# Horizon1026/Feature_Tracker

Hardware: AMD Instinct MI355X
Metric: tracked features/sec (2000 pts, 640x480, 4-lvl pyr) (higher is better)
Workload: dtype f32; 1 GPU; config2: basic KLT inverse, 2000 features/GPU, 640x480, 4-level pyramid, 21x21 patch; parallelism=single GPU

## Files before the change

feature_tracker_amd/csrc/ftk_device.h:

```cpp
#pragma once

#include <hip/hip_runtime.h>
#include <stdint.h>

#include "../../include/ftk.h"

namespace ftk {

constexpr int kWave = 64;

constexpr int kAffineTermsGroupFloats = 4 * 24 + 4;
constexpr int kAffineTermsRoundGroups = 4;

struct DevImage {
    const uint8_t *data;
    int32_t rows;
    int32_t cols;
};

struct KltParams {
    DevImage ref[FTK_MAX_LEVELS];
    DevImage cur[FTK_MAX_LEVELS];
    int32_t n_levels;
    int32_t single_level;
// ... 23 lines not shown
    int32_t half_rows, half_cols;
    float converge;
    float prior[4];
    int32_t consider_luminance;
    int32_t patch_rows, patch_cols, P, Ppad;
    int32_t ex_rows, ex_cols, E;
    int32_t a0_floats;
    uint32_t magic_pc;
    uint32_t magic_pc20;
    uint32_t magic_exc;
    int32_t rwin_rows, rwin_cols;
    int32_t cwin_rows, cwin_cols, cwin_margin;
    uint32_t magic_rwc, magic_cwc;
    uint32_t magic_rwq, magic_cwq;
    int32_t waves_per_feature;
    int32_t px_floats;
    int32_t quad_chain;
    int32_t terms_floats;
    int32_t lssd_chunked;
    int32_t features_per_group;
    int32_t group_lds_stride;
    int32_t pb_enabled;
    int32_t pb_rwin_rows, pb_rwin_cols;
    uint32_t pb_magic_rwc, pb_magic_rwq;
    int32_t pb_cap_r, pb_cap_c;
    int32_t fk_enabled;
    int32_t spill;
    float *spill_base;
    uint32_t spill_stride_floats;
    int32_t tree;
    int32_t scale_recip;
};

__host__ __device__ constexpr uint32_t klt_div_magic(int32_t d) { return d <= 1 ? 0u : (uint32_t)(((1ull << 32) + (uint64_t)d - 1) / (uint64_t)d); }

__host__ __device__ constexpr void klt_fill_geometry(KltParams &p) {
    p.patch_rows = 2 * p.half_rows + 1;
    p.patch_cols = 2 * p.half_cols + 1;
    p.P = p.patch_rows * p.patch_cols;
    p.Ppad = (p.P + 15) & ~15;
    p.ex_rows = p.patch_rows + 2;
    p.ex_cols = p.patch_cols + 2;
    p.E = p.ex_rows * p.ex_cols;
    const int32_t epad = (p.E + 3) & ~3, tables = 12 * (p.patch_rows + p.patch_cols);
    p.a0_floats = epad > tables ? epad : tables;
    p.magic_pc = klt_div_magic(p.patch_cols);
    p.magic_pc20 = (p.patch_cols > 1 && (long long)p.P * p.patch_cols < (1ll << 20) && p.P < (1 << 12))
                       ? (uint32_t)(((1u << 20) + (uint32_t)p.patch_cols - 1) / (uint32_t)p.patch_cols) : 0u;
    p.magic_exc = klt_div_magic(p.ex_cols);
    p.rwin_rows = p.patch_rows + 3;
    p.rwin_cols = (p.patch_cols + 3 + 3) & ~3;
    p.cwin_margin = 2;
    p.cwin_rows = p.rwin_rows + 2 * p.cwin_margin;
    p.cwin_cols = (p.patch_cols + 3 + 2 * p.cwin_margin + 3) & ~3;
    p.magic_rwc = klt_div_magic(p.rwin_cols);
    p.magic_cwc = klt_div_magic(p.cwin_cols);
    p.magic_rwq = klt_div_magic(p.rwin_cols / 4);
    p.magic_cwq = klt_div_magic(p.cwin_cols / 4);
    p.pb_rwin_rows = p.patch_rows + 4;
    p.pb_rwin_cols = (p.patch_cols + 4 + 3) & ~3;
    p.pb_magic_rwc = klt_div_magic(p.pb_rwin_cols);
    p.pb_magic_rwq = klt_div_magic(p.pb_rwin_cols / 4);
    int bits_r = 0, bits_c = 0;
    while ((1 << bits_r) < p.patch_rows + 2) {
        ++bits_r;
    }
    while ((1 << bits_c) < p.patch_cols + 2) {
        ++bits_c;
    }
    p.pb_cap_r = p.patch_rows + 2 + 2 * (bits_r + 3);
    p.pb_cap_c = p.patch_cols + 2 + 2 * (bits_c + 3);
}

hipError_t klt_position_order_launch(const float *ref_uv, int32_t n, const uint32_t *last_table, uint32_t last_call, uint8_t *pred, uint32_t *hist_and_cursor,
                                     int32_t *order, hipStream_t stream);
hipError_t ldlt6_launch(const float *d_a, const float *d_b, float *d_x, int n, hipStream_t stream);

constexpr int kMatchBlock = 256;
constexpr int kMatchRefs = 2;
constexpr int kMatchRowsPerBlock = kMatchBlock * kMatchRefs;
constexpr int kMfmaRows = 64;
constexpr int kMfmaTile = 32;
constexpr int kMfmaMaxTilesPerSplit = 1024;
constexpr long long kSmallMatchWork = 32ll << 20;
constexpr int kSmallMatchRowWork = 24576;
constexpr int kSmallNoIndex = 0xFFFFF;

struct MatchParams {
    const uint32_t *ref_words;
    const uint32_t *cur_words;
    const float *pred_uv;
    const float *cur_uv;
    int32_t *index_pairs;
    unsigned long long *keys;
// ... 371 lines not shown
```

feature_tracker_amd/csrc/klt_basic_kernels.hip:

```cpp
#define FTK_CHAIN_ROUND 4
#include "klt_common.h"
#include "klt_plan.h"

namespace ftk {
namespace {

constexpr int kChunk = 64;
constexpr bool pb_row_chunks(int patch_rows, int patch_cols) {
    if (patch_rows < 1 || patch_cols < 1 || patch_cols > kChunk) {
        return false;
    }
    const int rows_per_chunk = kChunk / patch_cols;
    return (patch_rows + rows_per_chunk - 1) / rows_per_chunk == (patch_rows * patch_cols + kChunk - 1) / kChunk;
}
template <int HR, int HC>
struct PbChunks {
    static constexpr int kRows = HR > 0 && HC > 0 ? 2 * HR + 1 : 0, kCols = HR > 0 && HC > 0 ? 2 * HC + 1 : 0;
    static constexpr bool kByRows = pb_row_chunks(kRows, kCols);
    static constexpr int kRowsPerChunk = kByRows ? kChunk / kCols : 1;
    static constexpr int kCount = kByRows ? (kRows + kRowsPerChunk - 1) / kRowsPerChunk : 0;
    static constexpr bool kLastRowsShort = kCount * kRowsPerChunk > kRows;
};
static_assert(PbChunks<10, 10>::kByRows && PbChunks<10, 10>::kCount == 7 && !PbChunks<10, 10>::kLastRowsShort, "21 x 21: seven chunks of three rows");
static_assert(!PbChunks<6, 6>::kByRows && !PbChunks<5, 5>::kByRows && !PbChunks<0, 0>::kByRows, "13 x 13, 11 x 11 and the run-time geometry stay linear");
constexpr int kRingRow = kChunk + 16;
constexpr int kTerms = 5;
constexpr int kCurQuads = 4;
constexpr int kRefQuads = 3;

__host__ __device__ inline int pb_pad4(int x) { return (x + 3) & ~3; }
__host__ __device__ inline int pb_producers(int waves) { return waves > 1 ? waves - 1 : 1; }
__host__ __device__ inline int pb_ring_slots(int waves) { return waves > 1 ? 2 : 1; }

struct PbLds {
    float4 *rnodes, *cnodes;
    uint4 *ridx, *cidx;
    float4 *ctab;
    float *ring;
    float *lattice;
    float *sol;
    uint32_t *slots;
    uint16_t *ref_win;
    int ref_win_stride;
    uint16_t *cur_win;
};

__host__ __device__ inline int pb_tables(const KltParams &p, int waves) { return p.tree ? waves : pb_producers(waves); }

__host__ __device__ inline size_t pb_lds_bytes(const KltParams &p, int waves) {
    const int np = pb_producers(waves);
    size_t bytes = 16 * (size_t)(p.pb_cap_r + p.pb_cap_c);
    bytes += 16 * (size_t)(p.patch_rows + p.patch_cols);
    bytes += 16 * (size_t)pb_tables(p, waves) * 2 * (p.patch_rows + p.patch_cols);
    bytes += 4 * (size_t)pb_ring_slots(waves) * np * kTerms * kRingRow;
    bytes += 4 * (size_t)pb_pad4(p.pb_cap_r * p.pb_cap_c);
    bytes += 4 * 4 + 4 * 16;
    bytes += 2 * (size_t)2 * pb_pad4(p.pb_rwin_rows * p.pb_rwin_cols);
    bytes += 2 * (size_t)pb_pad4(p.cwin_rows * p.cwin_cols);
    return (bytes + 15) & ~(size_t)15;
}

__device__ __forceinline__ PbLds pb_carve(float4 *base, const KltParams &p, int waves) {
    const int np = pb_producers(waves);
    PbLds c;
    c.rnodes = base;
    c.cnodes = c.rnodes + p.pb_cap_r;
    c.ridx = reinterpret_cast<uint4 *>(c.cnodes + p.pb_cap_c);
    c.cidx = c.ridx + p.patch_rows;
    c.ctab = reinterpret_cast<float4 *>(c.cidx + p.patch_cols);
    c.ring = reinterpret_cast<float *>(c.ctab + pb_tables(p, waves) * 2 * (p.patch_rows + p.patch_cols));
    c.lattice = c.ring + pb_ring_slots(waves) * np * kTerms * kRingRow;
    c.sol = c.lattice + pb_pad4(p.pb_cap_r * p.pb_cap_c);
    c.slots = reinterpret_cast<uint32_t *>(c.sol + 4);
    c.ref_win = reinterpret_cast<uint16_t *>(c.slots + 16);
    c.ref_win_stride = pb_pad4(p.pb_rwin_rows * p.pb_rwin_cols);
    c.cur_win = c.ref_win + 2 * c.ref_win_stride;
    return c;
}

__device__ __forceinline__ float4 node_entry(float x, int limit, int lo, int extent, int pitch) {
    const Axis a = make_axis(x, limit);
    const int rel = (int)((unsigned)a.i0 - (unsigned)lo);
    const bool hit = (unsigned)rel < (unsigned)extent;
    return make_float4(__int_as_float(hit ? rel * pitch : 0), a.sub, a.inv, __int_as_float((a.valid && hit) ? 1 : 0));
}

struct AxisSpec {
    int len, h, limit, lo, extent, pitch, cap;
    float centre;
    float4 *nodes;
    uint4 *idx;
    uint32_t *n_out;
};

__device__ __forceinline__ void build_nodes_pass(int lane, const AxisSpec &A, const AxisSpec &B) {
    const bool is_b = lane >= A.len;
    const int len = is_b ? B.len : A.len;
    const int h = is_b ? B.h : A.h;
// ... 36 lines not shown
        if (t == 0 || t == len - 1) {
            nodes[t == 0 ? 0 : len + 1] = node_entry(t == 0 ? xm : xp, limit, lo, extent, pitch);
        }
        const int im = (t == 0) ? 0 : (needm ? em : t);
        const int ip = (t == len - 1) ? len + 1 : (needp ? ep : t + 2);
        idx[t] = make_uint4((unsigned)(t + 1), (unsigned)im, (unsigned)ip, (v0 && vm && vp) ? 1u : 0u);
        if (t == 0) {
            *(is_b ? B.n_out : A.n_out) = (uint32_t)total;
        }
    }
    if (len == 1 && act) {
        nodes[2] = node_entry(xp, limit, lo, extent, pitch);
    }
    if ((bm | bp) != 0ull) {
        if (needm) {
            nodes[em] = node_entry(xm, limit, lo, extent, pitch);
        }
        if (needp) {
            nodes[ep] = node_entry(xp, limit, lo, extent, pitch);
        }
    }
}

__device__ __forceinline__ float node_tap(const uint16_t *win, int wcols, const float4 &nr, const float4 &nc) {
    const int idx = __float_as_int(nr.x) + __float_as_int(nc.x);
    const unsigned a = win[idx];
    const unsigned bb = win[idx + wcols];
    const float w_tl = nr.z * nc.z;
    const float w_tr = nr.z * nc.y;
    const float w_bl = nr.y * nc.z;
    const float w_br = nr.y * nc.y;
    return w_tl * (float)(a & 0xFFu) + w_tr * (float)(a >> 8) + w_bl * (float)(bb & 0xFFu) + w_br * (float)(bb >> 8);
}

__device__ __forceinline__ void cur_tables(int lane, const KltParams &p, const PbLds &c, float4 *tab, const DevImage &cur, const Win &cw, float cur_u,
                                           float cur_v, int n_c) {
    const int total = p.patch_rows + p.patch_cols;
    for (int t = lane; t < total; t += kWave) {
        const bool is_row = t < p.patch_rows;
        const int d = is_row ? t : t - p.patch_rows;
        const float x = (float)(d - (is_row ? p.half_rows : p.half_cols)) + (is_row ? cur_v : cur_u);
        float4 e = node_entry(x, (is_row ? cur.rows : cur.cols) - 1, is_row ? cw.r_lo : cw.c_lo, is_row ? cw.rows - 1 : cw.cols,
                              is_row ? cw.cols : 1);
        const uint4 id = is_row ? c.ridx[d] : c.cidx[d];
        e.w = __int_as_float(__float_as_int(e.w) & (int)id.w);
        const int mul = is_row ? n_c : 1;
        tab[t] = e;
        tab[total + t] = make_float4(__int_as_float((int)id.x * mul), __int_as_float((int)id.y * mul), __int_as_float((int)id.z * mul), 0.0f);
    }
}

struct PbLane {
    int row, col;
    bool in;
};
struct PbCols {
    float4 c0, c1;
};
template <class G>
__device__ __forceinline__ PbLane pb_lane(int lane) {
    PbLane l = {0, 0, false};
    if constexpr (G::kByRows) {
        constexpr uint32_t kMagic = (1048576 + G::kCols - 1) / G::kCols;
        const int row = (int)(__umul24((uint32_t)lane, kMagic) >> 20);
        l.in = lane < G::kRowsPerChunk * G::kCols;
        l.row = l.in ? row : 0;
        l.col = l.in ? lane - row * G::kCols : 0;
    }
    return l;
}
template <class G>
__device__ __forceinline__ void pb_read_cols(const PbLane &l, const KltParams &p, const float4 *tab, PbCols &cols) {
    if constexpr (G::kByRows) {
        cols.c0 = tab[p.patch_rows + l.col];
        cols.c1 = tab[2 * p.patch_rows + p.patch_cols + l.col];
    }
}

template <class G>
__device__ __forceinline__ bool chunk_products(int lane, int chunk, const KltParams &p, const PbLds &c, const float4 *tab, const Win &cw, const PbLane &l,
                                               const PbCols &cols, float (&prod)[kTerms]) {
    const int tab_total = p.patch_rows + p.patch_cols;
    bool in;
    float4 r0, r1, c0, c1;
    if constexpr (G::kByRows) {
        int prow = wadd(l.row, imul(chunk, G::kRowsPerChunk));
        in = l.in;
        if constexpr (G::kLastRowsShort) {
            in = in && prow < p.patch_rows;
            prow = in ? prow : 0;
        }
        r0 = tab[prow];
        r1 = tab[tab_total + prow];
        c0 = cols.c0;
        c1 = cols.c1;
    } else {
        const int pxi = chunk * kChunk + lane;
        in = pxi < p.P;
        const int pp = in ? pxi : 0;
        int prow, pcol;
        pixel_rc(p, pp, prow, pcol);
        r0 = tab[prow];
        r1 = tab[tab_total + prow];
        c0 = tab[p.patch_rows + pcol];
        c1 = tab[tab_total + p.patch_rows + pcol];
    }
    const float i_cur = node_tap(cw.data, cw.cols, r0, c0);
    const float *lat = c.lattice;
    const int rc = __float_as_int(r1.x), rm = __float_as_int(r1.y), rp = __float_as_int(r1.z);
    const int cc = __float_as_int(c1.x), cm = __float_as_int(c1.y), cp = __float_as_int(c1.z);
    const float left = lat[rc + cm];
    const float right = lat[rc + cp];
    const float top = lat[rm + cc];
    const float bottom = lat[rp + cc];
    const float i_ref = lat[rc + cc];
    const bool ok = in && ((__float_as_int(r0.w) & __float_as_int(c0.w)) != 0);
    const float fx = ok ? right - left : 0.0f;
    const float fy = ok ? bottom - top : 0.0f;
    const float ft = ok ? i_cur - i_ref : 0.0f;
    prod[0] = fx * fx;
    prod[1] = fy * fy;
    prod[2] = fx * fy;
    prod[3] = -(fx * ft);
    prod[4] = -(fy * ft);
    return ok;
}

template <class G>
__device__ __forceinline__ bool produce_chunk(int lane, int chunk, const KltParams &p, const PbLds &c, const float4 *tab, const Win &cw, const PbLane &l,
                                              const PbCols &cols, float *slot) {
    float prod[kTerms];
    const bool ok = chunk_products<G>(lane, chunk, p, c, tab, cw, l, cols, prod);
#pragma unroll
    for (int k = 0; k < kTerms; ++k) {
        slot[k * kRingRow + lane] = prod[k];
    }
    return ok;
}

__device__ __forceinline__ void wave_sum5(float (&v)[kTerms]) {
#pragma unroll
    for (int off = 32; off >= 1; off >>= 1) {
#pragma unroll
        for (int k = 0; k < kTerms; ++k) {
            v[k] += __shfl_xor(v[k], off, kWave);
        }
    }
}

__device__ __forceinline__ uint32_t magic20(int d) {
    uint32_t m = (uint32_t)(1048576.0f / (float)d);
    while (m * (uint32_t)d < 1048576u) {
        ++m;
    }
    return m;
}

constexpr int kWavesPerEu = 4;

__device__ __forceinline__ bool pb_window_inside(const DevImage &im, int r_lo, int c_lo, int wrows, int wcols) {
    return r_lo >= 0 && c_lo >= 0 && r_lo <= im.rows - wrows && c_lo <= im.cols - wcols - 4;
}

__device__ __forceinline__ void pb_sync(bool solo) {
    if (solo) {
        __builtin_amdgcn_fence(__ATOMIC_ACQ_REL, "wavefront");
        __builtin_amdgcn_wave_barrier();
    } else {
        __syncthreads();
    }
}

template <bool SOLO, int HR, int HC, bool TREE>
__global__ void __attribute__((amdgpu_waves_per_eu(kWavesPerEu))) __launch_bounds__(256) klt_basic_inverse_pipelined_kernel(const KltParams p_arg) {
    klt_touch_kernarg<sizeof(KltParams)>();
    KltParams p = p_arg;
    if constexpr (HR > 0 && HC > 0) {
        p.half_rows = HR;
        p.half_cols = HC;
        klt_fill_geometry(p);
    }
    extern __shared__ float4 lds_raw[];
    Blk b;
    uint32_t id;
    float4 *lds_mine = lds_raw;
    uint32_t block = blockIdx.x;
    if (p.sort_iters) {
        if (block == 0) {
            klt_order_block(p.sort_iters, p.sort_order_out, p.n, reinterpret_cast<int *>(lds_raw), p.sort_ref_uv, p_arg.ref[0].cols, p_arg.ref[0].rows, SOLO ? max(p.features_per_group, 1) : 1,
                            p.sched_flags, p.sched_call);
            return;
        }
        block -= 1;
    }
    if (SOLO) {
        b.tid = b.lane = threadIdx.x & (kWave - 1);
        b.nt = kWave;
        b.wave = 0;
        b.nwaves = 1;
        const uint32_t slot = threadIdx.x >> 6;
        id = block * (uint32_t)p.features_per_group + slot;
        lds_mine = lds_raw + (size_t)slot * (p.group_lds_stride >> 4);
    } else {
        b.tid = threadIdx.x;
// ... 60 lines not shown
    const bool last_chunk_short = !G::kByRows && p.P - (n_chunks - 1) * kChunk <= 48;
    const float *const quad_rows = c.ring + min(b.lane >> 2, kTerms - 1) * kRingRow + 4 * (b.lane & 3);

    const float full_ref_u = full_ref.x, full_ref_v = full_ref.y;
    const float scale = p.single_level ? 1.0f : (float)(1 << (p.n_levels - 1));
    float ref_u = full_ref_u, ref_v = full_ref_v, cur_u = in_u, cur_v = in_v;
    if (!p.single_level) {
        const uint32_t k = (uint32_t)(p.n_levels - 1);
        const float inv_scale = __uint_as_float((127u - k) << 23), least = __uint_as_float((1u + k) << 23);
        const bool normal = fabsf(full_ref_u) >= least && fabsf(full_ref_v) >= least && fabsf(in_u) >= least && fabsf(in_v) >= least;
        if (p.scale_recip && wave_ballot(!normal) == 0ull) {
            ref_u = full_ref_u * inv_scale;
            ref_v = full_ref_v * inv_scale;
            cur_u = in_u * inv_scale;
            cur_v = in_v * inv_scale;
        } else {
            ref_u = full_ref_u / scale;
            ref_v = full_ref_v / scale;
            cur_u = in_u / scale;
            cur_v = in_v / scale;
        }
    }

    const int rrows = p.pb_rwin_rows, rcols = p.pb_rwin_cols;
    const int ref_quads_total = rrows * (rcols >> 2), cur_quads_total = p.cwin_rows * (p.cwin_cols >> 2);
    const bool ref_fits = ref_quads_total <= kRefQuads * b.nt, cur_fits = cur_quads_total <= kCurQuads * b.nt;

    int buf = 0;
    int ref_r_lo, ref_c_lo;
    {
        const DevImage ref = p_arg.ref[p.n_levels - 1];
        footprint_origin(p, ref_u, ref_v, ref_r_lo, ref_c_lo);
        stage_any(opaque_blk(b), ref, c.ref_win, ref_r_lo, ref_c_lo, rrows, rcols, p.pb_magic_rwc, p.pb_magic_rwq);
    }
    uint32_t iters = 0;
    float out_u = in_u, out_v = in_v;
    const int base_n_c = p.patch_cols + 2;
    const uint32_t base_magic = (HC > 0) ? (uint32_t)((1048576 + base_n_c - 1) / base_n_c) : magic20(base_n_c);
    for (int level = p.n_levels - 1; level > -1; --level) {
        const DevImage ref = p_arg.ref[level];
        const DevImage cur = p_arg.cur[level];
        set_level_priority(level, younger);
        Win rw, cw;
        rw.data = c.ref_win + buf * c.ref_win_stride;
        rw.rows = rrows;
        rw.cols = rcols;
        rw.r_lo = ref_r_lo;
        rw.c_lo = ref_c_lo;
        int need_r, need_c;
        footprint_origin(p, cur_u, cur_v, need_r, need_c);
        cw.data = c.cur_win;
        cw.r_lo = wadd(need_r, -p.cwin_margin);
        cw.c_lo = wadd(need_c, -p.cwin_margin);
        cw.rows = p.cwin_rows;
        cw.cols = p.cwin_cols;
        win_set_cover(p, cw);
        int nr_lo = 0, nc_lo = 0;
        if (level > 0) {
            footprint_origin(p, ref_u * 2.0f, ref_v * 2.0f, nr_lo, nc_lo);
        }
        const bool cur_async = cur_fits && pb_window_inside(cur, cw.r_lo, cw.c_lo, cw.rows, cw.cols);
        const bool next_async = level > 0 && ref_fits && pb_window_inside(p_arg.ref[level > 0 ? level - 1 : 0], nr_lo, nc_lo, rrows, rcols);
        RawQuads<kCurQuads> qc;
        RawQuads<kRefQuads> qn;
        if (cur_async) {
            issue_quads(qc, b, cur, cw.r_lo, cw.c_lo, cw.rows, cw.cols, p.magic_cwq);
        }
        if (next_async) {
            issue_quads(qn, b, p_arg.ref[level - 1], nr_lo, nc_lo, rrows, rcols, p.pb_magic_rwq);
        }
        if (b.wave == 0) {
            AxisSpec ar = {p.patch_rows, p.half_rows, ref.rows - 1, rw.r_lo, rw.rows - 1, rw.cols, p.pb_cap_r, ref_v, c.rnodes, c.ridx, &c.slots[0]};
            AxisSpec ac = {p.patch_cols, p.half_cols, ref.cols - 1, rw.c_lo, rw.cols, 1, p.pb_cap_c, ref_u, c.cnodes, c.cidx, &c.slots[1]};
            const int lane = opaque(b.lane);
            if (p.patch_rows + p.patch_cols <= kWave) {
                build_nodes_pass(lane, ar, ac);
            } else {
                AxisSpec none = ar;
                none.len = 0;
                build_nodes_pass(lane, ar, none);
                build_nodes_pass(lane, ac, none);
            }
        }
        pb_sync(solo);
        const int n_r = __builtin_amdgcn_readfirstlane((int)c.slots[0]), n_c = __builtin_amdgcn_readfirstlane((int)c.slots[1]);
        {
            const int total = n_r * n_c;
            const uint32_t m = (n_c == base_n_c) ? base_magic : magic20(n_c);
            for (int idx = opaque(b.tid); idx < total; idx += b.nt) {
                const int r = (int)(__umul24((uint32_t)idx, m) >> 20);
                const int cc = idx - imul(r, n_c);
                c.lattice[idx] = node_tap(rw.data, rw.cols, c.rnodes[r], c.cnodes[cc]);
            }
        }
        if (cur_async) {
            store_quads(qc, b, c.cur_win, cw.rows, cw.cols, p.magic_cwq);
        } else {
            stage_any(opaque_blk(b), cur, c.cur_win, cw.r_lo, cw.c_lo, cw.rows, cw.cols, p.magic_cwc, p.magic_cwq);
        }
        if (level > 0) {
            if (next_async) {
                store_quads(qn, b, c.ref_win + (buf ^ 1) * c.ref_win_stride, rrows, rcols, p.pb_magic_rwq);
            } else {
                stage_any(opaque_blk(b), p_arg.ref[level - 1], c.ref_win + (buf ^ 1) * c.ref_win_stride, nr_lo, nc_lo, rrows, rcols, p.pb_magic_rwc, p.pb_magic_rwq);
            }
        }
        pb_sync(solo);

        for (uint32_t iter = 0; iter < p.max_iteration; ++iter) {
            ++iters;
            if (iter > 0 && !win_covers(cw, cur_u, cur_v)) {
                footprint_origin(p, cur_u, cur_v, need_r, need_c);
                const long long nr = need_r, nc = need_c;
                const bool covered = nr >= (long long)cw.r_lo && nr + (2 * p.half_rows + 4) <= (long long)cw.r_lo + cw.rows &&
                                     nc >= (long long)cw.c_lo && nc + (2 * p.half_cols + 4) <= (long long)cw.c_lo + cw.cols + 1;
                if (!covered) {
                    cw.r_lo = wadd(need_r, -p.cwin_margin);
                    cw.c_lo = wadd(need_c, -p.cwin_margin);
                    win_set_cover(p, cw);
                    stage_any(opaque_blk(b), cur, c.cur_win, cw.r_lo, cw.c_lo, cw.rows, cw.cols, p.magic_cwc, p.magic_cwq);
                    pb_sync(solo);
                }
            }
            uint32_t wave_valid = 0;
            float acc = 0.0f;
            PbCols my_cols = {};
            if constexpr (TREE) {
                float part[kTerms] = {0.0f, 0.0f, 0.0f, 0.0f, 0.0f};
                cur_tables(b.lane, p, c, my_tab, cur, cw, cur_u, cur_v, n_c);
                __builtin_amdgcn_wave_barrier();
                pb_read_cols<G>(my_px, p, my_tab, my_cols);
                for (int chunk = b.wave; chunk < n_chunks; chunk += b.nwaves) {
                    float prod[kTerms];
                    const bool ok = chunk_products<G>(b.lane, chunk, p, c, my_tab, cw, my_px, my_cols, prod);
#pragma unroll
                    for (int k = 0; k < kTerms; ++k) {
                        part[k] += prod[k];
                    }
                    wave_valid += (uint32_t)__popcll(wave_ballot(ok));
                }
                wave_sum5(part);
                float *const wave_sums = c.ring;
                if (b.lane == 0) {
// ... 121 lines not shown
        if (p.iters) {
            p.iters[id] = iters;
        }
        tail_report(p, iters, id);
        sched_grid_record(p, full_ref_u, full_ref_v, out_u, out_v, iters);
        if (p.sched_iters) {
            p.sched_iters[id] = iters;
        }
    }
}


}

namespace {
template <int HR, int HC>
KltKernel pick_kernel(bool solo, bool tree) {
    void (*entry)(const KltParams);
    if (tree) {
        entry = solo ? klt_basic_inverse_pipelined_kernel<true, HR, HC, true> : klt_basic_inverse_pipelined_kernel<false, HR, HC, true>;
    } else {
        entry = solo ? klt_basic_inverse_pipelined_kernel<true, HR, HC, false> : klt_basic_inverse_pipelined_kernel<false, HR, HC, false>;
    }
    return {entry, "pipelined", HR, solo, tree, false, false, PbChunks<HR, HC>::kByRows};
}
}

size_t klt_pipelined_feature_lds_bytes(const KltParams &p) { return pb_lds_bytes(p, p.waves_per_feature); }

KltKernel klt_pipelined_pick(const KltParams &p) {
    const bool solo = p.waves_per_feature == 1;
    if (p.half_rows == p.half_cols) {
        KltParams check = p;
        klt_fill_geometry(check);
        const bool same = check.pb_cap_r == p.pb_cap_r && check.pb_cap_c == p.pb_cap_c && check.cwin_rows == p.cwin_rows && check.cwin_cols == p.cwin_cols;
        if (same) {
            switch (p.half_rows) {
                case 5: return pick_kernel<5, 5>(solo, p.tree != 0);
                case 6: return pick_kernel<6, 6>(solo, p.tree != 0);
                case 10: return pick_kernel<10, 10>(solo, p.tree != 0);
                default: break;
            }
        }
    }
    return pick_kernel<0, 0>(solo, p.tree != 0);
}

__global__ void klt_basic_warm_kernel() {}
hipError_t klt_basic_warm(hipStream_t stream) {
    hipLaunchKernelGGL(klt_basic_warm_kernel, dim3(1), dim3(64), 0, stream);
    return hipGetLastError();
}

}
```

feature_tracker_amd/csrc/klt_common.h:

```cpp
#pragma once

#include "ftk_device.h"
#include "klt_sched.h"

#include <limits.h>
#include <math.h>
#include <stddef.h>

#include <type_traits>

namespace ftk {
namespace {



__device__ __forceinline__ int f2i(float x) { return (x >= -2147483648.0f && x < 2147483648.0f) ? (int)x : INT_MIN; }
__device__ __forceinline__ int wadd(int a, int b) { return (int)((unsigned)a + (unsigned)b); }
__device__ __forceinline__ int imul(int a, int b) { return __mul24(a, b); }
__device__ __forceinline__ unsigned long long wave_ballot(bool pred) { return __builtin_amdgcn_ballot_w64(pred); }
__device__ __forceinline__ float floor_from_trunc(float x, int t) {
    const float f = (float)t;
    return (f > x) ? f - 1.0f : f;
}
__device__ __forceinline__ float px(const DevImage &im, int row, int col) { return (float)im.data[__umul24((unsigned)row, (unsigned)im.cols) + (unsigned)col]; }
// ... 929 lines not shown
template <bool kBlocks64 = false>
__device__ __forceinline__ float chain_quads_row(float acc, const float *quad_row, int n16) {
    return chain_quads_strided<kBlocks64>(acc, reinterpret_cast<const float4 *>(quad_row), n16, 4);
}

constexpr int kChunkPixels = 64;
constexpr int kChunkRow = kChunkPixels + 4;

__device__ __forceinline__ void pixel_rc(const KltParams &p, int pxi, int &prow, int &pcol) {
    if (p.magic_pc20 != 0) {
        prow = (int)(__umul24((unsigned)pxi, p.magic_pc20) >> 20);
    } else {
        prow = (p.patch_cols == 1) ? pxi : (int)__umulhi((unsigned)pxi, p.magic_pc);
    }
    pcol = pxi - imul(prow, p.patch_cols);
}


__device__ __forceinline__ void footprint_origin(const KltParams &p, float u, float v, int &r_lo, int &c_lo) {
    r_lo = __builtin_amdgcn_readfirstlane(wadd(f2i(floorf(v)), -(p.half_rows + 1)));
    c_lo = __builtin_amdgcn_readfirstlane(wadd(f2i(floorf(u)), -(p.half_cols + 1)));
}

__device__ __forceinline__ void win_set_cover(const KltParams &p, Win &w) {
    const bool small = (unsigned)(w.r_lo + (1 << 22)) < (1u << 23) && (unsigned)(w.c_lo + (1 << 22)) < (1u << 23);
    w.cover[0] = small ? (float)(w.r_lo + p.half_rows + 1) : 1.0f;
    w.cover[1] = small ? (float)(w.r_lo + w.rows - p.half_rows - 3) : 0.0f;
    w.cover[2] = small ? (float)(w.c_lo + p.half_cols + 1) : 1.0f;
    w.cover[3] = small ? (float)(w.c_lo + w.cols - p.half_cols - 2) : 0.0f;
}

__device__ __forceinline__ bool win_covers(const Win &w, float u, float v) {
    const float fu = floorf(u), fv = floorf(v);
    return fv >= w.cover[0] && fv <= w.cover[1] && fu >= w.cover[2] && fu <= w.cover[3];
}

__device__ __forceinline__ uint16_t window_element(const DevImage &im, int r_lo, int c_lo, int idx, int wcols, uint32_t magic_cols) {
    const int r = (int)__umulhi((unsigned)idx, magic_cols);
    const int c = idx - imul(r, wcols);
    const int ir = clampi(wadd(r_lo, r), 0, im.rows - 1);
    const int ic = wadd(c_lo, c);
    const int ic0 = clampi(ic, 0, im.cols - 1);
    const int ic1 = clampi(wadd(ic, 1), 0, im.cols - 1);
    const unsigned row_off = __umul24((unsigned)ir, (unsigned)im.cols);
    return (uint16_t)((unsigned)im.data[row_off + (unsigned)ic0] | ((unsigned)im.data[row_off + (unsigned)ic1] << 8));
}

constexpr int kStageBatch = 4;

__device__ __forceinline__ void stage_elements(const Blk &b, const DevImage &im, uint16_t *dst, int r_lo, int c_lo, int wcols, uint32_t magic_cols,
                                               int total) {
    for (int base = 0; base < total; base += b.nt * kStageBatch) {
        uint16_t v[kStageBatch];
#pragma unroll
        for (int k = 0; k < kStageBatch; ++k) {
// ... 101 lines not shown
}

template <int N>
__device__ __forceinline__ void store_quads(const RawQuads<N> &q, const Blk &b, uint16_t *dst, int wrows, int wcols, uint32_t magic_quads) {
    const int quads = wcols >> 2;
    const int total = wrows * quads;
    const int tid = opaque(b.tid);
#pragma unroll
    for (int k = 0; k < N; ++k) {
        const int idx = tid + k * b.nt;
        if (idx < total) {
            const int r = (quads == 1) ? idx : (int)__umulhi((unsigned)idx, magic_quads);
            const int qq = idx - imul(r, quads);
            const uint32_t x = q.x[k], y = q.y[k];
            const uint32_t p0 = x & 0xFFFFu;
            const uint32_t p1 = (x >> 8) & 0xFFFFu;
            const uint32_t p2 = x >> 16;
            const uint32_t p3 = __builtin_amdgcn_alignbyte(y, x, 3) & 0xFFFFu;
            *reinterpret_cast<uint2 *>(dst + imul(r, wcols) + 4 * qq) = make_uint2(p0 | (p1 << 16), p2 | (p3 << 16));
        }
    }
}

}


__device__ __forceinline__ uint32_t sched_table_slot(float u, float v) {
    const uint32_t qx = (uint32_t)(int)fminf(fmaxf(u * 0.25f, 0.0f), 1048575.0f), qy = (uint32_t)(int)fminf(fmaxf(v * 0.25f, 0.0f), 1048575.0f);
    return ((qx * 73856093u) ^ (qy * 19349663u)) & (uint32_t)(kSchedTableSize - 1);
}

__device__ __forceinline__ uint32_t sched_prediction(const KltParams &p, float u, float v) {
    const uint32_t word = p.sched_grid[(((p.sched_call - 1u) & 1u) << kSchedTableBits) + sched_table_slot(u, v)];
    return sched_grid_call(word) == sched_grid_tag(p.sched_call - 1u) ? sched_grid_iters(word) : 0u;
}

__device__ __forceinline__ void sched_grid_record(const KltParams &p, float ref_u, float ref_v, float out_u, float out_v, uint32_t iters) {
    if (p.sched_grid != nullptr) {
        const uint32_t word = sched_grid_pack(p.sched_call, iters);
        uint32_t *table = p.sched_grid + sched_table_at(p.sched_call);
        const uint32_t at_ref = sched_table_slot(ref_u, ref_v), at_out = sched_table_slot(out_u, out_v);
        atomicMax(&table[at_ref], word);
        if (at_out != at_ref) {
            atomicMax(&table[at_out], word);
        }
    }
// ... 258 lines not shown
```

feature_tracker_amd/csrc/klt_plan.cpp:

```cpp
#include "klt_plan.h"

#include <algorithm>

namespace ftk {
namespace {
#include "klt_wave_policy.inc"

int policy_bucket(const int *centres, int count, int x) {
    int best = 0;
    for (int i = 1; i < count; ++i) {
        if ((long long)x * x > (long long)centres[i - 1] * centres[i]) {
            best = i;
        }
    }
    return best;
}

int clamp_1_4(int x) { return x < 1 ? 1 : (x > 4 ? 4 : x); }

bool fast_like(int method) { return method != FTK_METHOD_INVERSE && method != FTK_METHOD_DIRECT; }

bool affine_terms(const KltPlanInput &in) { return in.model == FTK_MODEL_AFFINE && !fast_like(in.method); }

int32_t affine_terms_floats(const KltParams &p) {
    return ((p.Ppad / 4 + kAffineTermsRoundGroups - 1) / kAffineTermsRoundGroups) * kAffineTermsRoundGroups * kAffineTermsGroupFloats;
}

int plan_waves(const KltPlanInput &in, int pixels) {
    int waves = klt_policy_waves(in.model, klt_method_class(in.method), in.consider_luminance, in.long_tail, pixels, in.n);
    if (in.tree && waves == 1 && fast_like(in.method) && in.model != FTK_MODEL_LSSD) {
        waves = std::min(4, std::max(2, (pixels + 63) / 64));
    }
    return in.waves != kKltNotSet ? in.waves : clamp_1_4(waves);
}

int plan_group(const KltPlanInput &in, int waves, int measured_best) {
    if (waves != 1) {
        return 1;
    }
    return in.group != kKltNotSet ? in.group : measured_best;
}

KltForm pick_form(const KltPlanInput &in, const KltParams &geometry, int waves) {
    const bool exact_coordinates = in.max_extent < (1 << 23);
    if (in.model == FTK_MODEL_BASIC && in.method == FTK_METHOD_INVERSE && geometry.patch_rows <= 64 && geometry.patch_cols <= 64 && exact_coordinates) {
        return KltForm::Pipelined;
    }
    const bool fast_model = in.model == FTK_MODEL_BASIC || in.model == FTK_MODEL_AFFINE;
    if (fast_model && fast_like(in.method) && !in.tree && waves == 1 && geometry.P <= 1024 && exact_coordinates &&
        klt_fast_feature_lds_bytes(in.model, geometry) <= 40 * 1024) {
        return KltForm::OneWaveFast;
    }
    return KltForm::Generic;
}

size_t shape_in_lds(const KltPlanInput &in, KltForm form, int waves, KltParams &p) {
    p.tree = in.tree;
    p.waves_per_feature = waves;
    p.px_floats = 3;
    p.terms_floats = 0;
    p.lssd_chunked = 0;
    size_t one = 0;
    if (form == KltForm::Pipelined) {
        p.pb_enabled = 1;
        p.features_per_group = plan_group(in, waves, 4);
        one = klt_pipelined_feature_lds_bytes(p);
    } else if (form == KltForm::OneWaveFast) {
        p.fk_enabled = 1;
// ... 90 lines not shown
```

feature_tracker_amd/csrc/klt_plan.h:

```cpp
#pragma once

#include "ftk_device.h"
#include "klt_sched.h"

namespace ftk {

struct KltPlanInput {
    int model, method;
    int32_t half_rows, half_cols;
    int32_t n;
    int32_t max_extent;
    int consider_luminance;
    int tree;
    int long_tail;
    int waves, group, lssd_chunked, spill;
};

enum class KltForm {
    Pipelined,
    OneWaveFast,
    Generic,
    GenericSpill,
};

// ... 2 lines not shown
    size_t lds_bytes;
    unsigned grid, block;
};

enum KltPlanError { kKltPlanOk = 0, kKltPlanUnknownVariant, kKltPlanSpillTooLarge };

KltPlanError klt_plan(const KltPlanInput &in, KltParams *p, KltPlan *plan, size_t *spill_floats);

int klt_policy_waves(int model, int method_class, int consider_luminance, int long_tail, int pixels, int n);

size_t klt_pipelined_feature_lds_bytes(const KltParams &p);
size_t klt_fast_feature_lds_bytes(int model, const KltParams &p);
size_t klt_generic_feature_lds_bytes(int model, const KltParams &p);
size_t klt_spill_lds_bytes(int model, const KltParams &p);
size_t klt_spill_floats(int model, const KltParams &p);

struct KltKernel {
    void (*entry)(const KltParams);
    const char *family;
    int half;
    bool solo;
    bool tree, lum, spill;
    bool row_chunks = false;
};
KltKernel klt_pipelined_pick(const KltParams &p);
KltKernel klt_fast_pick(int model, const KltParams &p);
KltKernel klt_pick(const KltPlan &plan, int model, int method, const KltParams &p);

hipError_t klt_launch(const KltPlan &plan, int model, int method, const KltParams &p, hipStream_t stream);

}
```

Measured before the change: 58.23 million tracked features/s.

## Stage pipelined KLT windows as raw bytes with power-of-two pitch

Image windows in LDS change from uint16-widened pixels to raw uint8 rows padded to a power-of-two pitch. They are copied as 8-byte units using shift/mask addressing instead of magic-number division. Bilinear taps now read two aligned words per row and extract the bytes with alignbyte. The aim is to halve LDS traffic for window staging and cheapen address math. In exchange, tap reads cost extra ALU for byte extraction, and the inside-image check needs the full pitch to lie within the image, so windows near the edge fall back to the slower clamped path more often.

```diff
diff --git a/feature_tracker_amd/csrc/ftk_device.h b/feature_tracker_amd/csrc/ftk_device.h
--- a/feature_tracker_amd/csrc/ftk_device.h
+++ b/feature_tracker_amd/csrc/ftk_device.h
@@ -69,7 +69,6 @@
     int32_t group_lds_stride;
     int32_t pb_enabled;
     int32_t pb_rwin_rows, pb_rwin_cols;
-    uint32_t pb_magic_rwc, pb_magic_rwq;
     int32_t pb_cap_r, pb_cap_c;
     int32_t fk_enabled;
     int32_t spill;
@@ -77,9 +76,33 @@
     uint32_t spill_stride_floats;
     int32_t tree;
     int32_t scale_recip;
+    int32_t pb_rwin_pitch, pb_cwin_pitch;
 };
 
 __host__ __device__ constexpr uint32_t klt_div_magic(int32_t d) { return d <= 1 ? 0u : (uint32_t)(((1ull << 32) + (uint64_t)d - 1) / (uint64_t)d); }
+
+__host__ __device__ constexpr int32_t klt_byte_window_room(int32_t rows, int32_t cols) { return 2 * ((rows * cols + 3) & ~3); }
+__host__ __device__ constexpr int32_t klt_byte_pitch(int32_t cols) {
+    const int32_t pitch8 = (cols + 1 + 7) & ~7;
+    int32_t pow2 = 8;
+    while (pow2 < pitch8) {
+        pow2 *= 2;
+    }
+    return pow2;
+}
+__host__ __device__ constexpr uint32_t klt_byte_unit_offset(uint32_t idx, int shift, uint32_t im_cols) {
+    return (idx >> shift) * im_cols + 8u * (idx & ((1u << shift) - 1u));
+}
+__host__ __device__ constexpr int klt_byte_units_shift(int32_t pitch) {
+    int shift = 0;
+    while ((8 << shift) < pitch) {
+        ++shift;
+    }
+    return shift;
+}
+__host__ __device__ constexpr bool klt_byte_window_inside(int32_t im_rows, int32_t im_cols, int32_t r_lo, int32_t c_lo, int32_t wrows, int32_t pitch) {
+    return r_lo >= 0 && c_lo >= 0 && r_lo <= im_rows - wrows && c_lo <= im_cols - pitch;
+}
 
 __host__ __device__ constexpr void klt_fill_geometry(KltParams &p) {
     p.patch_rows = 2 * p.half_rows + 1;
@@ -106,8 +129,8 @@
     p.magic_cwq = klt_div_magic(p.cwin_cols / 4);
     p.pb_rwin_rows = p.patch_rows + 4;
     p.pb_rwin_cols = (p.patch_cols + 4 + 3) & ~3;
-    p.pb_magic_rwc = klt_div_magic(p.pb_rwin_cols);
-    p.pb_magic_rwq = klt_div_magic(p.pb_rwin_cols / 4);
+    p.pb_rwin_pitch = klt_byte_pitch(p.pb_rwin_cols);
+    p.pb_cwin_pitch = klt_byte_pitch(p.cwin_cols);
     int bits_r = 0, bits_c = 0;
     while ((1 << bits_r) < p.patch_rows + 2) {
         ++bits_r;
@@ -117,6 +140,13 @@
     }
     p.pb_cap_r = p.patch_rows + 2 + 2 * (bits_r + 3);
     p.pb_cap_c = p.patch_cols + 2 + 2 * (bits_c + 3);
+}
+
+__host__ __device__ constexpr bool klt_byte_window_ok(int32_t rows, int32_t cols, int32_t pitch) {
+    return pitch >= cols + 1 && (pitch & (pitch - 1)) == 0 && pitch % 8 == 0 && rows * pitch <= klt_byte_window_room(rows, cols);
+}
+__host__ __device__ constexpr bool klt_byte_windows_ok(const KltParams &p) {
+    return klt_byte_window_ok(p.pb_rwin_rows, p.pb_rwin_cols, p.pb_rwin_pitch) && klt_byte_window_ok(p.cwin_rows, p.cwin_cols, p.pb_cwin_pitch);
 }
 
 hipError_t klt_position_order_launch(const float *ref_uv, int32_t n, const uint32_t *last_table, uint32_t last_call, uint8_t *pred, uint32_t *hist_and_cursor,
diff --git a/feature_tracker_amd/csrc/klt_basic_kernels.hip b/feature_tracker_amd/csrc/klt_basic_kernels.hip
--- a/feature_tracker_amd/csrc/klt_basic_kernels.hip
+++ b/feature_tracker_amd/csrc/klt_basic_kernels.hip
@@ -25,8 +25,10 @@
 static_assert(!PbChunks<6, 6>::kByRows && !PbChunks<5, 5>::kByRows && !PbChunks<0, 0>::kByRows, "13 x 13, 11 x 11 and the run-time geometry stay linear");
 constexpr int kRingRow = kChunk + 16;
 constexpr int kTerms = 5;
-constexpr int kCurQuads = 4;
-constexpr int kRefQuads = 3;
+constexpr int kRunTimeRefOctets = 3, kRunTimeCurOctets = 4;
+constexpr int pb_octets(int rows, int pitch, bool solo, int run_time) {
+    return rows > 0 ? (rows * (pitch / 8) + (solo ? 64 : 128) - 1) / (solo ? 64 : 128) : run_time;
+}
 
 __host__ __device__ inline int pb_pad4(int x) { return (x + 3) & ~3; }
 __host__ __device__ inline int pb_producers(int waves) { return waves > 1 ? waves - 1 : 1; }
@@ -40,9 +42,9 @@
     float *lattice;
     float *sol;
     uint32_t *slots;
-    uint16_t *ref_win;
+    uint8_t *ref_win;
     int ref_win_stride;
-    uint16_t *cur_win;
+    uint8_t *cur_win;
 };
 
 __host__ __device__ inline int pb_tables(const KltParams &p, int waves) { return p.tree ? waves : pb_producers(waves); }
@@ -72,8 +74,8 @@
     c.lattice = c.ring + pb_ring_slots(waves) * np * kTerms * kRingRow;
     c.sol = c.lattice + pb_pad4(p.pb_cap_r * p.pb_cap_c);
     c.slots = reinterpret_cast<uint32_t *>(c.sol + 4);
-    c.ref_win = reinterpret_cast<uint16_t *>(c.slots + 16);
-    c.ref_win_stride = pb_pad4(p.pb_rwin_rows * p.pb_rwin_cols);
+    c.ref_win = reinterpret_cast<uint8_t *>(c.slots + 16);
+    c.ref_win_stride = 2 * pb_pad4(p.pb_rwin_rows * p.pb_rwin_cols);
     c.cur_win = c.ref_win + 2 * c.ref_win_stride;
     return c;
 }
@@ -156,18 +158,28 @@
     }
 }
 
-__device__ __forceinline__ float node_tap(const uint16_t *win, int wcols, const float4 &nr, const float4 &nc) {
+struct PbWin {
+    const uint8_t *data;
+    int r_lo, c_lo;
+    int rows, cols, pitch;
+    float cover[4];
+};
+
+__device__ __forceinline__ float node_tap(const uint8_t *win, int pitch, const float4 &nr, const float4 &nc) {
     const int idx = __float_as_int(nr.x) + __float_as_int(nc.x);
-    const unsigned a = win[idx];
-    const unsigned bb = win[idx + wcols];
+    const uint32_t *const w = reinterpret_cast<const uint32_t *>(win) + (idx >> 2);
+    const uint32_t top = __builtin_amdgcn_alignbyte(w[1], w[0], (uint32_t)idx & 3u);
+    const uint32_t bot = __builtin_amdgcn_alignbyte(w[(pitch >> 2) + 1], w[pitch >> 2], (uint32_t)idx & 3u);
+    const unsigned tl = top & 0xFFu, tr = (top >> 8) & 0xFFu;
+    const unsigned bl = bot & 0xFFu, br = (bot >> 8) & 0xFFu;
     const float w_tl = nr.z * nc.z;
     const float w_tr = nr.z * nc.y;
     const float w_bl = nr.y * nc.z;
     const float w_br = nr.y * nc.y;
-    return w_tl * (float)(a & 0xFFu) + w_tr * (float)(a >> 8) + w_bl * (float)(bb & 0xFFu) + w_br * (float)(bb >> 8);
-}
-
-__device__ __forceinline__ void cur_tables(int lane, const KltParams &p, const PbLds &c, float4 *tab, const DevImage &cur, const Win &cw, float cur_u,
+    return w_tl * (float)tl + w_tr * (float)tr + w_bl * (float)bl + w_br * (float)br;
+}
+
+__device__ __forceinline__ void cur_tables(int lane, const KltParams &p, const PbLds &c, float4 *tab, const DevImage &cur, const PbWin &cw, float cur_u,
                                            float cur_v, int n_c) {
     const int total = p.patch_rows + p.patch_cols;
     for (int t = lane; t < total; t += kWave) {
@@ -175,7 +187,7 @@
         const int d = is_row ? t : t - p.patch_rows;
         const float x = (float)(d - (is_row ? p.half_rows : p.half_cols)) + (is_row ? cur_v : cur_u);
         float4 e = node_entry(x, (is_row ? cur.rows : cur.cols) - 1, is_row ? cw.r_lo : cw.c_lo, is_row ? cw.rows - 1 : cw.cols,
-                              is_row ? cw.cols : 1);
+                              is_row ? cw.pitch : 1);
         const uint4 id = is_row ? c.ridx[d] : c.cidx[d];
         e.w = __int_as_float(__float_as_int(e.w) & (int)id.w);
         const int mul = is_row ? n_c : 1;
@@ -212,7 +224,7 @@
 }
 
 template <class G>
-__device__ __forceinline__ bool chunk_products(int lane, int chunk, const KltParams &p, const PbLds &c, const float4 *tab, const Win &cw, const PbLane &l,
+__device__ __forceinline__ bool chunk_products(int lane, int chunk, const KltParams &p, const PbLds &c, const float4 *tab, const PbWin &cw, const PbLane &l,
                                                const PbCols &cols, float (&prod)[kTerms]) {
     const int tab_total = p.patch_rows + p.patch_cols;
     bool in;
@@ -239,7 +251,7 @@
         c0 = tab[p.patch_rows + pcol];
         c1 = tab[tab_total + p.patch_rows + pcol];
     }
-    const float i_cur = node_tap(cw.data, cw.cols, r0, c0);
+    const float i_cur = node_tap(cw.data, cw.pitch, r0, c0);
     const float *lat = c.lattice;
     const int rc = __float_as_int(r1.x), rm = __float_as_int(r1.y), rp = __float_as_int(r1.z);
     const int cc = __float_as_int(c1.x), cm = __float_as_int(c1.y), cp = __float_as_int(c1.z);
@@ -261,7 +273,7 @@
 }
 
 template <class G>
-__device__ __forceinline__ bool produce_chunk(int lane, int chunk, const KltParams &p, const PbLds &c, const float4 *tab, const Win &cw, const PbLane &l,
+__device__ __forceinline__ bool produce_chunk(int lane, int chunk, const KltParams &p, const PbLds &c, const float4 *tab, const PbWin &cw, const PbLane &l,
                                               const PbCols &cols, float *slot) {
     float prod[kTerms];
     const bool ok = chunk_products<G>(lane, chunk, p, c, tab, cw, l, cols, prod);
@@ -292,8 +304,16 @@
 
 constexpr int kWavesPerEu = 4;
 
-__device__ __forceinline__ bool pb_window_inside(const DevImage &im, int r_lo, int c_lo, int wrows, int wcols) {
-    return r_lo >= 0 && c_lo >= 0 && r_lo <= im.rows - wrows && c_lo <= im.cols - wcols - 4;
+constexpr KltParams pb_geometry(int hr, int hc) {
+    KltParams g = {};
+    g.half_rows = hr;
+    g.half_cols = hc;
+    klt_fill_geometry(g);
+    return g;
+}
+
+__device__ __forceinline__ bool pb_window_inside(const DevImage &im, int r_lo, int c_lo, int wrows, int pitch) {
+    return klt_byte_window_inside(im.rows, im.cols, r_lo, c_lo, wrows, pitch);
 }
 
 __device__ __forceinline__ void pb_sync(bool solo) {
@@ -314,6 +334,10 @@
         p.half_cols = HC;
         klt_fill_geometry(p);
     }
+    constexpr KltParams kGeo = pb_geometry(HR, HC);
+    static_assert(HR == 0 || klt_byte_windows_ok(kGeo), "byte windows: power-of-two pitch inside the carved regions");
+    constexpr int kCurOctets = pb_octets(HR > 0 ? kGeo.cwin_rows : 0, kGeo.pb_cwin_pitch, SOLO, kRunTimeCurOctets);
+    constexpr int kRefOctets = pb_octets(HR > 0 ? kGeo.pb_rwin_rows : 0, kGeo.pb_rwin_pitch, SOLO, kRunTimeRefOctets);
     extern __shared__ float4 lds_raw[];
     Blk b;
     uint32_t id;
@@ -420,16 +444,15 @@
         }
     }
 
-    const int rrows = p.pb_rwin_rows, rcols = p.pb_rwin_cols;
-    const int ref_quads_total = rrows * (rcols >> 2), cur_quads_total = p.cwin_rows * (p.cwin_cols >> 2);
-    const bool ref_fits = ref_quads_total <= kRefQuads * b.nt, cur_fits = cur_quads_total <= kCurQuads * b.nt;
+    const int rrows = p.pb_rwin_rows, rcols = p.pb_rwin_cols, rpitch = p.pb_rwin_pitch, cpitch = p.pb_cwin_pitch;
+    const bool ref_fits = rrows * (rpitch >> 3) <= kRefOctets * b.nt, cur_fits = p.cwin_rows * (cpitch >> 3) <= kCurOctets * b.nt;
 
     int buf = 0;
     int ref_r_lo, ref_c_lo;
     {
         const DevImage ref = p_arg.ref[p.n_levels - 1];
         footprint_origin(p, ref_u, ref_v, ref_r_lo, ref_c_lo);
-        stage_any(opaque_blk(b), ref, c.ref_win, ref_r_lo, ref_c_lo, rrows, rcols, p.pb_magic_rwc, p.pb_magic_rwq);
+        stage_bytes_any(opaque_blk(b), ref, c.ref_win, ref_r_lo, ref_c_lo, rrows, rpitch);
     }
     uint32_t iters = 0;
     float out_u = in_u, out_v = in_v;
@@ -439,10 +462,11 @@
         const DevImage ref = p_arg.ref[level];
         const DevImage cur = p_arg.cur[level];
         set_level_priority(level, younger);
-        Win rw, cw;
+        PbWin rw, cw;
         rw.data = c.ref_win + buf * c.ref_win_stride;
         rw.rows = rrows;
         rw.cols = rcols;
+        rw.pitch = rpitch;
         rw.r_lo = ref_r_lo;
         rw.c_lo = ref_c_lo;
         int need_r, need_c;
@@ -452,23 +476,24 @@
         cw.c_lo = wadd(need_c, -p.cwin_margin);
         cw.rows = p.cwin_rows;
         cw.cols = p.cwin_cols;
+        cw.pitch = cpitch;
         win_set_cover(p, cw);
         int nr_lo = 0, nc_lo = 0;
         if (level > 0) {
             footprint_origin(p, ref_u * 2.0f, ref_v * 2.0f, nr_lo, nc_lo);
         }
-        const bool cur_async = cur_fits && pb_window_inside(cur, cw.r_lo, cw.c_lo, cw.rows, cw.cols);
-        const bool next_async = level > 0 && ref_fits && pb_window_inside(p_arg.ref[level > 0 ? level - 1 : 0], nr_lo, nc_lo, rrows, rcols);
-        RawQuads<kCurQuads> qc;
-        RawQuads<kRefQuads> qn;
+        const bool cur_async = cur_fits && pb_window_inside(cur, cw.r_lo, cw.c_lo, cw.rows, cpitch);
+        const bool next_async = level > 0 && ref_fits && pb_window_inside(p_arg.ref[level > 0 ? level - 1 : 0], nr_lo, nc_lo, rrows, rpitch);
+        RawOctets<kCurOctets> qc;
+        RawOctets<kRefOctets> qn;
         if (cur_async) {
-            issue_quads(qc, b, cur, cw.r_lo, cw.c_lo, cw.rows, cw.cols, p.magic_cwq);
+            issue_octets(qc, b, cur, cw.r_lo, cw.c_lo, cw.rows, cpitch);
         }
         if (next_async) {
-            issue_quads(qn, b, p_arg.ref[level - 1], nr_lo, nc_lo, rrows, rcols, p.pb_magic_rwq);
+            issue_octets(qn, b, p_arg.ref[level - 1], nr_lo, nc_lo, rrows, rpitch);
         }
         if (b.wave == 0) {
-            AxisSpec ar = {p.patch_rows, p.half_rows, ref.rows - 1, rw.r_lo, rw.rows - 1, rw.cols, p.pb_cap_r, ref_v, c.rnodes, c.ridx, &c.slots[0]};
+            AxisSpec ar = {p.patch_rows, p.half_rows, ref.rows - 1, rw.r_lo, rw.rows - 1, rw.pitch, p.pb_cap_r, ref_v, c.rnodes, c.ridx, &c.slots[0]};
             AxisSpec ac = {p.patch_cols, p.half_cols, ref.cols - 1, rw.c_lo, rw.cols, 1, p.pb_cap_c, ref_u, c.cnodes, c.cidx, &c.slots[1]};
             const int lane = opaque(b.lane);
             if (p.patch_rows + p.patch_cols <= kWave) {
@@ -488,19 +513,19 @@
             for (int idx = opaque(b.tid); idx < total; idx += b.nt) {
                 const int r = (int)(__umul24((uint32_t)idx, m) >> 20);
                 const int cc = idx - imul(r, n_c);
-                c.lattice[idx] = node_tap(rw.data, rw.cols, c.rnodes[r], c.cnodes[cc]);
+                c.lattice[idx] = node_tap(rw.data, rw.pitch, c.rnodes[r], c.cnodes[cc]);
             }
         }
         if (cur_async) {
-            store_quads(qc, b, c.cur_win, cw.rows, cw.cols, p.magic_cwq);
+            store_octets(qc, b, c.cur_win, cw.rows, cpitch);
         } else {
-            stage_any(opaque_blk(b), cur, c.cur_win, cw.r_lo, cw.c_lo, cw.rows, cw.cols, p.magic_cwc, p.magic_cwq);
+            stage_bytes_any(opaque_blk(b), cur, c.cur_win, cw.r_lo, cw.c_lo, cw.rows, cpitch);
         }
         if (level > 0) {
             if (next_async) {
-                store_quads(qn, b, c.ref_win + (buf ^ 1) * c.ref_win_stride, rrows, rcols, p.pb_magic_rwq);
+                store_octets(qn, b, c.ref_win + (buf ^ 1) * c.ref_win_stride, rrows, rpitch);
             } else {
-                stage_any(opaque_blk(b), p_arg.ref[level - 1], c.ref_win + (buf ^ 1) * c.ref_win_stride, nr_lo, nc_lo, rrows, rcols, p.pb_magic_rwc, p.pb_magic_rwq);
+                stage_bytes_any(opaque_blk(b), p_arg.ref[level - 1], c.ref_win + (buf ^ 1) * c.ref_win_stride, nr_lo, nc_lo, rrows, rpitch);
             }
         }
         pb_sync(solo);
@@ -516,7 +541,7 @@
                     cw.r_lo = wadd(need_r, -p.cwin_margin);
                     cw.c_lo = wadd(need_c, -p.cwin_margin);
                     win_set_cover(p, cw);
-                    stage_any(opaque_blk(b), cur, c.cur_win, cw.r_lo, cw.c_lo, cw.rows, cw.cols, p.magic_cwc, p.magic_cwq);
+                    stage_bytes_any(opaque_blk(b), cur, c.cur_win, cw.r_lo, cw.c_lo, cw.rows, cpitch);
                     pb_sync(solo);
                 }
             }
@@ -684,7 +709,9 @@
     } else {
         entry = solo ? klt_basic_inverse_pipelined_kernel<true, HR, HC, false> : klt_basic_inverse_pipelined_kernel<false, HR, HC, false>;
     }
-    return {entry, "pipelined", HR, solo, tree, false, false, PbChunks<HR, HC>::kByRows};
+    return {entry, "pipelined", HR, solo, tree, false, false, PbChunks<HR, HC>::kByRows,
+            pb_octets(HR > 0 ? pb_geometry(HR, HC).cwin_rows : 0, pb_geometry(HR, HC).pb_cwin_pitch, solo, kRunTimeCurOctets),
+            pb_octets(HR > 0 ? pb_geometry(HR, HC).pb_rwin_rows : 0, pb_geometry(HR, HC).pb_rwin_pitch, solo, kRunTimeRefOctets)};
 }
 }
 
@@ -695,7 +722,8 @@
     if (p.half_rows == p.half_cols) {
         KltParams check = p;
         klt_fill_geometry(check);
-        const bool same = check.pb_cap_r == p.pb_cap_r && check.pb_cap_c == p.pb_cap_c && check.cwin_rows == p.cwin_rows && check.cwin_cols == p.cwin_cols;
+        const bool same = check.pb_cap_r == p.pb_cap_r && check.pb_cap_c == p.pb_cap_c && check.cwin_rows == p.cwin_rows && check.cwin_cols == p.cwin_cols &&
+                          check.pb_rwin_pitch == p.pb_rwin_pitch && check.pb_cwin_pitch == p.pb_cwin_pitch;
         if (same) {
             switch (p.half_rows) {
                 case 5: return pick_kernel<5, 5>(solo, p.tree != 0);
diff --git a/feature_tracker_amd/csrc/klt_common.h b/feature_tracker_amd/csrc/klt_common.h
--- a/feature_tracker_amd/csrc/klt_common.h
+++ b/feature_tracker_amd/csrc/klt_common.h
@@ -975,7 +975,8 @@
     c_lo = __builtin_amdgcn_readfirstlane(wadd(f2i(floorf(u)), -(p.half_cols + 1)));
 }
 
-__device__ __forceinline__ void win_set_cover(const KltParams &p, Win &w) {
+template <class W>
+__device__ __forceinline__ void win_set_cover(const KltParams &p, W &w) {
     const bool small = (unsigned)(w.r_lo + (1 << 22)) < (1u << 23) && (unsigned)(w.c_lo + (1 << 22)) < (1u << 23);
     w.cover[0] = small ? (float)(w.r_lo + p.half_rows + 1) : 1.0f;
     w.cover[1] = small ? (float)(w.r_lo + w.rows - p.half_rows - 3) : 0.0f;
@@ -983,7 +984,8 @@
     w.cover[3] = small ? (float)(w.c_lo + w.cols - p.half_cols - 2) : 0.0f;
 }
 
-__device__ __forceinline__ bool win_covers(const Win &w, float u, float v) {
+template <class W>
+__device__ __forceinline__ bool win_covers(const W &w, float u, float v) {
     const float fu = floorf(u), fv = floorf(v);
     return fv >= w.cover[0] && fv <= w.cover[1] && fu >= w.cover[2] && fu <= w.cover[3];
 }
@@ -1131,6 +1133,102 @@
     }
 }
 
+__device__ __forceinline__ int byte_units_shift(int pitch) { return 28 - __builtin_clz((unsigned)pitch); }
+
+__device__ __forceinline__ unsigned byte_unit_offset(int idx, int shift, const DevImage &im) {
+    const unsigned r = (unsigned)idx >> shift, u = (unsigned)idx & ((1u << shift) - 1u);
+    return __umul24(r, (unsigned)im.cols) + 8u * u;
+}
+
+template <int N>
+struct RawOctets {
+    uint32_t x[N], y[N];
+};
+
+template <int N>
+__device__ __forceinline__ void issue_octets(RawOctets<N> &q, const Blk &b, const DevImage &im, int r_lo, int c_lo, int wrows, int pitch) {
+    const int shift = byte_units_shift(pitch);
+    const int total = wrows << shift;
+    const int tid = opaque(b.tid);
+    const uint8_t *base = im.data + (long long)r_lo * im.cols + c_lo;
+#pragma unroll
+    for (int k = 0; k < N; ++k) {
+        int idx = tid + k * b.nt;
+        idx = idx < total ? idx : 0;
+        const uint8_t *src = base + (size_t)byte_unit_offset(idx, shift, im);
+        __builtin_memcpy(&q.x[k], src, 4);
+        __builtin_memcpy(&q.y[k], src + 4, 4);
+    }
+}
+
+template <int N>
+__device__ __forceinline__ void store_octets(const RawOctets<N> &q, const Blk &b, uint8_t *dst, int wrows, int pitch) {
+    const int total = wrows << byte_units_shift(pitch);
+    const int tid = opaque(b.tid);
+#pragma unroll
+    for (int k = 0; k < N; ++k) {
+        const int idx = tid + k * b.nt;
+        if (idx < total) {
+            *reinterpret_cast<uint2 *>(dst + 8 * idx) = make_uint2(q.x[k], q.y[k]);
+        }
+    }
+}
+
+__device__ __forceinline__ void stage_bytes_inside(const Blk &b, const DevImage &im, uint8_t *dst, int r_lo, int c_lo, int wrows, int pitch) {
+    const int shift = byte_units_shift(pitch);
+    const int total = wrows << shift;
+    const uint8_t *base = im.data + (long long)r_lo * im.cols + c_lo;
+    for (int idx = b.tid; idx < total; idx += b.nt) {
+        const uint8_t *src = base + (size_t)byte_unit_offset(idx, shift, im);
+        uint32_t x, y;
+        __builtin_memcpy(&x, src, 4);
+        __builtin_memcpy(&y, src + 4, 4);
+        *reinterpret_cast<uint2 *>(dst + 8 * idx) = make_uint2(x, y);
+    }
+}
+
+__device__ __forceinline__ uint32_t byte_window_word(const DevImage &im, int r_lo, int c_lo, int word, int pitch_shift) {
+    const int r = word >> (pitch_shift - 2), c = (word & ((1 << (pitch_shift - 2)) - 1)) << 2;
+    const int ir = clampi(wadd(r_lo, r), 0, im.rows - 1);
+    const unsigned row_off = __umul24((unsigned)ir, (unsigned)im.cols);
+    uint32_t w = 0;
+#pragma unroll
+    for (int k = 0; k < 4; ++k) {
+        const int ic = clampi(wadd(c_lo, c + k), 0, im.cols - 1);
+        w |= (uint32_t)im.data[row_off + (unsigned)ic] << (8 * k);
+    }
+    return w;
+}
+
+__device__ __forceinline__ void stage_bytes_elements(const Blk &b, const DevImage &im, uint8_t *dst, int r_lo, int c_lo, int wrows, int pitch) {
+    const int pitch_shift = byte_units_shift(pitch) + 3;
+    const int total = wrows << (pitch_shift - 2);
+    uint32_t *const words = reinterpret_cast<uint32_t *>(dst);
+    for (int base = 0; base < total; base += b.nt * kStageBatch) {
+        uint32_t v[kStageBatch];
+#pragma unroll
+        for (int k = 0; k < kStageBatch; ++k) {
+            const int idx = base + k * b.nt + b.tid;
+            v[k] = byte_window_word(im, r_lo, c_lo, idx < total ? idx : 0, pitch_shift);
+        }
+#pragma unroll
+        for (int k = 0; k < kStageBatch; ++k) {
+            const int idx = base + k * b.nt + b.tid;
+            if (idx < total) {
+                words[idx] = v[k];
+            }
+        }
+    }
+}
+
+__device__ __forceinline__ void stage_bytes_any(const Blk &b, const DevImage &im, uint8_t *dst, int r_lo, int c_lo, int wrows, int pitch) {
+    if (klt_byte_window_inside(im.rows, im.cols, r_lo, c_lo, wrows, pitch)) {
+        stage_bytes_inside(b, im, dst, r_lo, c_lo, wrows, pitch);
+    } else {
+        stage_bytes_elements(b, im, dst, r_lo, c_lo, wrows, pitch);
+    }
+}
+
 }
 
 
diff --git a/feature_tracker_amd/csrc/klt_plan.cpp b/feature_tracker_amd/csrc/klt_plan.cpp
--- a/feature_tracker_amd/csrc/klt_plan.cpp
+++ b/feature_tracker_amd/csrc/klt_plan.cpp
@@ -43,7 +43,8 @@
 
 KltForm pick_form(const KltPlanInput &in, const KltParams &geometry, int waves) {
     const bool exact_coordinates = in.max_extent < (1 << 23);
-    if (in.model == FTK_MODEL_BASIC && in.method == FTK_METHOD_INVERSE && geometry.patch_rows <= 64 && geometry.patch_cols <= 64 && exact_coordinates) {
+    if (in.model == FTK_MODEL_BASIC && in.method == FTK_METHOD_INVERSE && geometry.patch_rows <= 64 && geometry.patch_cols <= 64 && exact_coordinates &&
+        klt_byte_windows_ok(geometry)) {
         return KltForm::Pipelined;
     }
     const bool fast_model = in.model == FTK_MODEL_BASIC || in.model == FTK_MODEL_AFFINE;
diff --git a/feature_tracker_amd/csrc/klt_plan.h b/feature_tracker_amd/csrc/klt_plan.h
--- a/feature_tracker_amd/csrc/klt_plan.h
+++ b/feature_tracker_amd/csrc/klt_plan.h
@@ -48,6 +48,7 @@
     bool solo;
     bool tree, lum, spill;
     bool row_chunks = false;
+    int cur_units = 0, ref_units = 0;
 };
 KltKernel klt_pipelined_pick(const KltParams &p);
 KltKernel klt_fast_pick(int model, const KltParams &p);
```

Result: faster. 61.52 million tracked features/s, median of 6 (+5.7%).
